# Zehong-Ma/MagCache

Hardware: NVIDIA H100
Metric: denoising_steps_per_sec (higher is better)
Workload: dtype bf16

## Files before the change

### magcache_b200/csrc/gemm_wgmma.cu

```cuda
#include <cstdlib>

#include "common.cuh"
#include "ptx.cuh"
#include "tma_host.cuh"

namespace mc {

TmapCacheEntry* tmap_cache() {
  static TmapCacheEntry table[kTmapCacheSize] = {};
  return table;
}
std::mutex& tmap_cache_mutex() {
  static std::mutex m;
  return m;
}

constexpr int kBM = 128, kBK = 64, kStages = 4;
constexpr int kTileABytes = kBM * kBK * 2;
constexpr int kStagePad = 33;
constexpr int kEpiWarps = 8;
constexpr int kStagingBytes = kEpiWarps * 32 * kStagePad * 4;
constexpr int kGemmThreads = 128 + 32 * kEpiWarps;
constexpr int kProducerRegs = 40, kConsumerRegs = 232;
template <int BN>
struct GemmTile {
  static constexpr int kTileBBytes = BN * kBK * 2;
  static constexpr int kStageBytes = kTileABytes + kTileBBytes;
  static constexpr int kOffStaging = kStages * kStageBytes;
  static constexpr int kOffBars = kOffStaging + kStagingBytes;
  static constexpr int kSmem = kOffBars + 128;
};

struct GemmParams {
  int M, N, K;
  const float* bias;
  void* out;
  int64_t ldo;
  const float* gate;
  int total_tiles;
};

template <int EPI>
__device__ __forceinline__ void epilogue_patch(const GemmParams& p, const float* stage, int row0, int col0, int lane) {
  const int rows = min(32, p.M - row0);
  if (rows <= 0) return;
  const int col = col0 + lane;
  const bool col_ok = col < p.N;

  if (EPI == MC_EPI_BIAS_GATE_RESID) {
    const float b = (p.bias && col_ok) ? p.bias[col] : 0.f;
    const float g = (p.gate && col_ok) ? p.gate[col] : 1.f;
    float* xcol = static_cast<float*>(p.out) + static_cast<int64_t>(row0) * p.ldo + col;
#pragma unroll
    for (int h = 0; h < 32; h += 16) {
      float xv[16];
#pragma unroll
      for (int r = 0; r < 16; ++r) xv[r] = (col_ok && h + r < rows) ? xcol[static_cast<int64_t>(h + r) * p.ldo] : 0.f;
#pragma unroll
      for (int r = 0; r < 16; ++r) {
        const float y = round_bf16(stage[(h + r) * kStagePad + lane] + b);
        xv[r] = __fadd_rn(xv[r], __fmul_rn(y, g));
      }
#pragma unroll
      for (int r = 0; r < 16; ++r)
        if (col_ok && h + r < rows) xcol[static_cast<int64_t>(h + r) * p.ldo] = xv[r];
    }
    return;
  }

  if (EPI == MC_EPI_BIAS_F32) {
    const float b = (p.bias && col_ok) ? p.bias[col] : 0.f;
    float* ocol = static_cast<float*>(p.out) + static_cast<int64_t>(row0) * p.ldo + col;
#pragma unroll
    for (int r = 0; r < 32; ++r)
      if (col_ok && r < rows) ocol[static_cast<int64_t>(r) * p.ldo] = stage[r * kStagePad + lane] + b;
    return;
  }

  const int half = lane >> 4, cp = (lane & 15) * 2;
  const int c0 = col0 + cp;
  float b0 = 0.f, b1 = 0.f;
  if (EPI != MC_EPI_ROWBIAS_BF16 && p.bias) {
    if (c0 < p.N) b0 = p.bias[c0];
    if (c0 + 1 < p.N) b1 = p.bias[c0 + 1];
  }
  float g0 = 1.f, g1 = 1.f;
  if (EPI == MC_EPI_BIAS_GATE_RESID_BF16 && p.gate) {
    if (c0 < p.N) g0 = p.gate[c0];
    if (c0 + 1 < p.N) g1 = p.gate[c0 + 1];
  }
  __nv_bfloat16* obase = static_cast<__nv_bfloat16*>(p.out) + static_cast<int64_t>(row0 + half) * p.ldo + c0;
  const float* sbase = stage + half * kStagePad + cp;
  const float* rbias = (EPI == MC_EPI_ROWBIAS_BF16 && p.bias) ? p.bias + row0 + half : nullptr;

  if (rows == 32 && col0 + 32 <= p.N && (p.ldo & 1) == 0) {
    uint32_t w[16];
#pragma unroll
    for (int i = 0; i < 16; ++i) {
      float v0 = sbase[2 * i * kStagePad], v1 = sbase[2 * i * kStagePad + 1];
      if (EPI == MC_EPI_ROWBIAS_BF16) {
        const float rb = rbias ? rbias[2 * i] : 0.f;
        v0 += rb;
        v1 += rb;
      } else {
        v0 += b0;
        v1 += b1;
      }
      if (EPI == MC_EPI_BIAS_GELU_BF16) {
        v0 = gelu_tanh(round_bf16(v0));
        v1 = gelu_tanh(round_bf16(v1));
      }
      if (EPI == MC_EPI_BIAS_GELU_ERF_BF16) {
        v0 = gelu_erf(round_bf16(v0));
        v1 = gelu_erf(round_bf16(v1));
      }
      if (EPI == MC_EPI_BIAS_SILU_BF16) {
        v0 = silu_f(round_bf16(v0));
        v1 = silu_f(round_bf16(v1));
      }
      if (EPI == MC_EPI_BIAS_GATE_RESID_BF16) {
        const uint32_t old = *reinterpret_cast<const uint32_t*>(obase + static_cast<int64_t>(2 * i) * p.ldo);
        v0 = bf16_lo(old) + round_bf16(g0 * round_bf16(v0));
        v1 = bf16_hi(old) + round_bf16(g1 * round_bf16(v1));
      }
      w[i] = pack_bf16x2(v0, v1);
    }
#pragma unroll
    for (int i = 0; i < 16; ++i) *reinterpret_cast<uint32_t*>(obase + static_cast<int64_t>(2 * i) * p.ldo) = w[i];
    return;
  }

  const bool pair_ok = (c0 + 1 < p.N) && ((p.ldo & 1) == 0);
  for (int i = 0; i < 16; ++i) {
    const int r = 2 * i + half;
    if (r >= rows) continue;
    float v0 = sbase[2 * i * kStagePad], v1 = sbase[2 * i * kStagePad + 1];
    if (EPI == MC_EPI_ROWBIAS_BF16) {
      const float rb = rbias ? rbias[2 * i] : 0.f;
      v0 += rb;
      v1 += rb;
    } else {
      v0 += b0;
      v1 += b1;
    }
    if (EPI == MC_EPI_BIAS_GELU_BF16) {
      v0 = gelu_tanh(round_bf16(v0));
      v1 = gelu_tanh(round_bf16(v1));
    }
    if (EPI == MC_EPI_BIAS_GELU_ERF_BF16) {
      v0 = gelu_erf(round_bf16(v0));
      v1 = gelu_erf(round_bf16(v1));
    }
    if (EPI == MC_EPI_BIAS_SILU_BF16) {
      v0 = silu_f(round_bf16(v0));
      v1 = silu_f(round_bf16(v1));
    }
    __nv_bfloat16* o = obase + static_cast<int64_t>(2 * i) * p.ldo;
    if (EPI == MC_EPI_BIAS_GATE_RESID_BF16) {
      if (c0 < p.N) v0 = __bfloat162float(o[0]) + round_bf16(g0 * round_bf16(v0));
      if (c0 + 1 < p.N) v1 = __bfloat162float(o[1]) + round_bf16(g1 * round_bf16(v1));
    }
    if (pair_ok) {
      *reinterpret_cast<uint32_t*>(o) = pack_bf16x2(v0, v1);
    } else {
      if (c0 < p.N) o[0] = __float2bfloat16_rn(v0);
      if (c0 + 1 < p.N) o[1] = __float2bfloat16_rn(v1);
    }
  }
}

template <int EPI, int kBN>
__global__ void __launch_bounds__(kGemmThreads, 1)
    gemm_bf16_kernel(const __grid_constant__ CUtensorMap tmap_a, const __grid_constant__ CUtensorMap tmap_b, const GemmParams p) {
  using T = GemmTile<kBN>;
  constexpr int kStageBytes = T::kStageBytes, kOffStaging = T::kOffStaging, kOffBars = T::kOffBars;
  extern __shared__ __align__(1024) uint8_t smem[];
  float* staging = reinterpret_cast<float*>(smem + kOffStaging);
  uint64_t* full_bar = reinterpret_cast<uint64_t*>(smem + kOffBars);
  uint64_t* empty_bar = full_bar + kStages;

  const int warp = threadIdx.x >> 5, lane = threadIdx.x & 31;
  const int n_tiles = (p.N + kBN - 1) / kBN;
  const int total_tiles = p.total_tiles;
  const int num_kb = (p.K + kBK - 1) / kBK;

  if (threadIdx.x == 0) {
    if ((ptx::smem_u32(smem) & 1023u) != 0) {
      MC_DIAG("gemm_bf16_kernel: dynamic smem base not 1024-aligned\n");
      __trap();
    }
    ptx::prefetch_tmap(&tmap_a);
    ptx::prefetch_tmap(&tmap_b);
    for (int s = 0; s < kStages; ++s) {
      ptx::mbar_init(&full_bar[s], 1);
      ptx::mbar_init(&empty_bar[s], kEpiWarps);
    }
    ptx::fence_mbar_init();
  }
  __syncthreads();

  if (warp < 4) {
    ptx::setmaxnreg_dec<kProducerRegs>();
    if (warp == 0) {
      uint32_t it = 0;
      for (int tile = blockIdx.x; tile < total_tiles; tile += gridDim.x) {
        const int m0 = (tile / n_tiles) * kBM, n0 = (tile % n_tiles) * kBN;
        for (int kb = 0; kb < num_kb; ++kb, ++it) {
          const int s = it % kStages;
          const uint32_t ph = (it / kStages) & 1;
          ptx::mbar_wait(&empty_bar[s], ph ^ 1);
          if (ptx::elect_one()) {
            uint8_t* sa = smem + s * kStageBytes;
            ptx::mbar_expect_tx(&full_bar[s], kStageBytes);
            ptx::tma_load_2d(sa, &tmap_a, &full_bar[s], kb * kBK, m0);
            ptx::tma_load_2d(sa + kTileABytes, &tmap_b, &full_bar[s], kb * kBK, n0);
          }
          __syncwarp();
        }
      }
    }
  } else {
    ptx::setmaxnreg_inc<kConsumerRegs>();
    const int wg = (warp >> 2) - 1;
    const int wq = warp & 3;
    float acc[kBN / 2];
    uint32_t it = 0;
    for (int tile = blockIdx.x; tile < total_tiles; tile += gridDim.x) {
      const int m0 = (tile / n_tiles) * kBM, n0 = (tile % n_tiles) * kBN;
      int prev_s = -1;
      for (int kb = 0; kb < num_kb; ++kb, ++it) {
        const int s = it % kStages;
        const uint32_t ph = (it / kStages) & 1;
        ptx::mbar_wait(&full_bar[s], ph);
        const uint32_t sa = ptx::smem_u32(smem + s * kStageBytes);
        const uint64_t da = ptx::gmma_desc_sw128_kmajor(sa + wg * (64 * 128));
        const uint64_t db = ptx::gmma_desc_sw128_kmajor(sa + kTileABytes);
        ptx::wgmma_fence();
#pragma unroll
        for (int k = 0; k < kBK / 16; ++k) {
          if constexpr (kBN == 256) {
            ptx::wgmma_m64n256k16_ss(acc, da + 2 * k, db + 2 * k, (kb | k) != 0 ? 1u : 0u);
          } else {
            ptx::wgmma_m64n128k16_ss(acc, da + 2 * k, db + 2 * k, (kb | k) != 0 ? 1u : 0u);
          }
        }
        ptx::wgmma_commit();
        ptx::wgmma_wait<1>();
        ptx::fence_regs(acc);
        if (prev_s >= 0 && lane == 0) ptx::mbar_arrive(&empty_bar[prev_s]);
        prev_s = s;
      }
      ptx::wgmma_wait<0>();
      ptx::fence_regs(acc);
      if (lane == 0) ptx::mbar_arrive(&empty_bar[prev_s]);

      const int pr = wq >> 1;
      const int row0 = m0 + wg * 64 + pr * 32;
      const int r_lo = (wq & 1) * 16 + (lane >> 2);
#pragma unroll
      for (int c = 0; c < kBN / 32; ++c) {
        float* patch = staging + (4 * wg + 2 * pr + (c & 1)) * 32 * kStagePad;
        asm volatile("bar.sync %0, 64;" ::"r"(1 + 2 * wg + pr) : "memory");
#pragma unroll
        for (int q = 0; q < 4; ++q) {
          const int i = 4 * c + q;
          const int col = 8 * q + 2 * (lane & 3);
          patch[r_lo * kStagePad + col] = acc[4 * i + 0];
          patch[r_lo * kStagePad + col + 1] = acc[4 * i + 1];
          patch[(r_lo + 8) * kStagePad + col] = acc[4 * i + 2];
          patch[(r_lo + 8) * kStagePad + col + 1] = acc[4 * i + 3];
        }
        asm volatile("bar.sync %0, 64;" ::"r"(1 + 2 * wg + pr) : "memory");
        if ((wq & 1) == (c & 1)) epilogue_patch<EPI>(p, patch, row0, n0 + c * 32, lane);
      }
    }
  }
}

template <int EPI, int BN>
static int32_t launch_gemm_bn(const CUtensorMap& ta, const CUtensorMap& tb, GemmParams p, cudaStream_t s) {
  static PerDeviceOnce once;
  const int32_t rc = set_max_smem_once(gemm_bf16_kernel<EPI, BN>, GemmTile<BN>::kSmem, once, "cudaFuncSetAttribute(gemm smem)");
  if (rc) return rc;
  const int m_tiles = (p.M + kBM - 1) / kBM, n_tiles = (p.N + BN - 1) / BN;
  const int total = m_tiles * n_tiles;
  p.total_tiles = total;
  const int grid = total < num_sms() ? total : num_sms();
  gemm_bf16_kernel<EPI, BN><<<grid, kGemmThreads, GemmTile<BN>::kSmem, s>>>(ta, tb, p);
  MC_CHECK_LAUNCH("gemm_bf16_kernel launch");
  return MC_OK;
}

static int pick_bn(int M, int N) {
  const char* e = getenv("MC_GEMM_BN");
  if (e && *e) {
    const int v = atoi(e);
    if (v == 128 || v == 256) return v;
  }
  const int64_t sms = num_sms(), m_tiles = (M + kBM - 1) / kBM;
  const int64_t t256 = m_tiles * ((N + 255) / 256), t128 = m_tiles * ((N + 127) / 128);
  const int64_t cost256 = ((t256 + sms - 1) / sms) * 100, cost128 = ((t128 + sms - 1) / sms) * 62;
  return cost128 * 100 <= cost256 * 92 ? 128 : 256;
}

}

extern "C" int32_t mc_gemm_bf16(const void* A, int64_t lda, const void* B, int64_t ldb, int32_t M, int32_t N, int32_t K,
                                const float* bias, int32_t epilogue, void* out, int64_t ldo, const float* gate, void* stream) {
  MC_CHECK_ARG(A && B && out, "mc_gemm_bf16: null pointer");
  MC_CHECK_ARG(M >= 1 && N >= 1 && K >= 8, "mc_gemm_bf16: M=%d N=%d K=%d", M, N, K);
  MC_CHECK_ARG(K % 8 == 0 && lda % 8 == 0 && ldb % 8 == 0 && lda >= K && ldb >= K, "mc_gemm_bf16: K/lda/ldb must be multiples of 8 (16-byte TMA pitch)");
  MC_CHECK_ARG(mc::aligned16(A) && mc::aligned16(B) && mc::aligned16(out), "mc_gemm_bf16: A/B/out must be 16-byte aligned");
  MC_CHECK_ARG(ldo >= N, "mc_gemm_bf16: ldo=%lld < N=%d", static_cast<long long>(ldo), N);
  CUtensorMap ta, tb;
  int32_t rc = mc::make_tmap_bf16_2d(&ta, A, static_cast<uint64_t>(M), static_cast<uint64_t>(K), static_cast<uint64_t>(lda), mc::kBM, mc::kBK);
  if (rc) return rc;
  const int bn = mc::pick_bn(M, N);
  rc = mc::make_tmap_bf16_2d(&tb, B, static_cast<uint64_t>(N), static_cast<uint64_t>(K), static_cast<uint64_t>(ldb), bn, mc::kBK);
  if (rc) return rc;
  mc::GemmParams p{M, N, K, bias, out, ldo, gate, 0};
  cudaStream_t s = static_cast<cudaStream_t>(stream);
#define MC_GEMM_CASE(E) \
  case E: return bn == 128 ? mc::launch_gemm_bn<E, 128>(ta, tb, p, s) : mc::launch_gemm_bn<E, 256>(ta, tb, p, s)
  switch (epilogue) {
    MC_GEMM_CASE(MC_EPI_BIAS_BF16);
    MC_GEMM_CASE(MC_EPI_BIAS_GELU_BF16);
    MC_GEMM_CASE(MC_EPI_BIAS_GATE_RESID);
    MC_GEMM_CASE(MC_EPI_ROWBIAS_BF16);
    MC_GEMM_CASE(MC_EPI_BIAS_F32);
    MC_GEMM_CASE(MC_EPI_BIAS_GELU_ERF_BF16);
    MC_GEMM_CASE(MC_EPI_BIAS_GATE_RESID_BF16);
    MC_GEMM_CASE(MC_EPI_BIAS_SILU_BF16);
#undef MC_GEMM_CASE
    default:
      mc::set_error("mc_gemm_bf16: unknown epilogue %d", epilogue);
      return MC_ERR_INVALID;
  }
}
```

### magcache_b200/csrc/ptx.cuh

```cuda
#pragma once
#include <cstdint>
#include <cuda_runtime.h>

namespace ptx {

__device__ __forceinline__ uint32_t smem_u32(const void* p) {
  return static_cast<uint32_t>(__cvta_generic_to_shared(p));
}

__device__ __forceinline__ void mbar_init(uint64_t* bar, uint32_t count) {
  asm volatile("mbarrier.init.shared::cta.b64 [%0], %1;" ::"r"(smem_u32(bar)), "r"(count) : "memory");
}
__device__ __forceinline__ void fence_mbar_init() {
  asm volatile("fence.mbarrier_init.release.cluster;" ::: "memory");
}
__device__ __forceinline__ void mbar_expect_tx(uint64_t* bar, uint32_t bytes) {
  asm volatile("mbarrier.arrive.expect_tx.shared::cta.b64 _, [%0], %1;" ::"r"(smem_u32(bar)), "r"(bytes) : "memory");
}
__device__ __forceinline__ void mbar_arrive(uint64_t* bar) {
  asm volatile("mbarrier.arrive.shared::cta.b64 _, [%0];" ::"r"(smem_u32(bar)) : "memory");
}
__device__ __forceinline__ bool mbar_try_wait(uint64_t* bar, uint32_t parity) {
  uint32_t ok;
  asm volatile(
      "{\n"
      ".reg .pred p;\n"
      "mbarrier.try_wait.parity.shared::cta.b64 p, [%1], %2;\n"
      "selp.u32 %0, 1, 0, p;\n"
      "}\n"
      : "=r"(ok)
      : "r"(smem_u32(bar)), "r"(parity)
      : "memory");
  return ok != 0;
}
#ifndef MC_DEVICE_DIAG
#define MC_DEVICE_DIAG 0
#endif
#if MC_DEVICE_DIAG
#define MC_DIAG(...) printf(__VA_ARGS__)
#else
#define MC_DIAG(...) ((void)0)
#endif

#ifndef MC_MBAR_TIMEOUT_CYCLES
#define MC_MBAR_TIMEOUT_CYCLES (4000000000ll)
#endif
__device__ __forceinline__ void mbar_wait(uint64_t* bar, uint32_t parity) {
  if (mbar_try_wait(bar, parity)) return;
  const long long t0 = clock64();
  while (!mbar_try_wait(bar, parity)) {
    if (clock64() - t0 > MC_MBAR_TIMEOUT_CYCLES) {
      MC_DIAG("mbar_wait timeout: block (%d,%d,%d) thread %d bar smem+%u parity %u\n", blockIdx.x, blockIdx.y, blockIdx.z,
              threadIdx.x, smem_u32(bar), parity);
      __trap();
    }
  }
}
__device__ __forceinline__ void mbar_wait_or_flag(uint64_t* bar, uint32_t parity, bool& timed_out) {
  if (timed_out || mbar_try_wait(bar, parity)) return;
  const long long t0 = clock64();
  while (!mbar_try_wait(bar, parity)) {
    if (clock64() - t0 > MC_MBAR_TIMEOUT_CYCLES) {
      MC_DIAG("mbar_wait timeout: block (%d,%d,%d) thread %d bar smem+%u parity %u\n", blockIdx.x, blockIdx.y, blockIdx.z,
              threadIdx.x, smem_u32(bar), parity);
      timed_out = true;
      return;
    }
  }
}

__device__ __forceinline__ void named_bar_sync(uint32_t id, uint32_t count) {
  asm volatile("bar.sync %0, %1;" ::"r"(id), "r"(count) : "memory");
}
__device__ __forceinline__ void named_bar_arrive(uint32_t id, uint32_t count) {
  asm volatile("bar.arrive %0, %1;" ::"r"(id), "r"(count) : "memory");
}

__device__ __forceinline__ bool elect_one() {
  uint32_t pred;
  asm volatile(
      "{\n"
      ".reg .pred P;\n"
      "elect.sync _|P, 0xffffffff;\n"
      "selp.u32 %0, 1, 0, P;\n"
      "}\n"
      : "=r"(pred));
  return pred != 0;
}

__device__ __forceinline__ void fence_proxy_async_smem() {
  asm volatile("fence.proxy.async.shared::cta;" ::: "memory");
}

__device__ __forceinline__ void prefetch_tmap(const void* tmap) {
  asm volatile("prefetch.tensormap [%0];" ::"l"(reinterpret_cast<uint64_t>(tmap)) : "memory");
}
__device__ __forceinline__ void tma_load_2d(void* smem_dst, const void* tmap, uint64_t* bar, int32_t c0, int32_t c1) {
  asm volatile(
      "cp.async.bulk.tensor.2d.shared::cluster.global.mbarrier::complete_tx::bytes [%0], [%1, {%3, %4}], [%2];"
      ::"r"(smem_u32(smem_dst)), "l"(reinterpret_cast<uint64_t>(tmap)), "r"(smem_u32(bar)), "r"(c0), "r"(c1)
      : "memory");
}

__device__ __forceinline__ void bulk_load_1d(void* smem_dst, const void* gmem_src, uint32_t bytes, uint64_t* bar) {
  asm volatile("cp.async.bulk.shared::cluster.global.mbarrier::complete_tx::bytes [%0], [%1], %2, [%3];" ::"r"(smem_u32(smem_dst)),
               "l"(reinterpret_cast<uint64_t>(gmem_src)), "r"(bytes), "r"(smem_u32(bar))
               : "memory");
}

__device__ __forceinline__ uint64_t gmma_desc_sw128_kmajor(uint32_t smem_addr) {
  uint64_t d = 0;
  d |= static_cast<uint64_t>((smem_addr & 0x3FFFFu) >> 4);
  d |= static_cast<uint64_t>(1) << 16;
  d |= static_cast<uint64_t>(1024 >> 4) << 32;
  d |= static_cast<uint64_t>(1) << 62;
  return d;
}
__device__ __forceinline__ uint64_t gmma_desc_sw128_mnmajor(uint32_t smem_addr, uint32_t lbo_bytes, uint32_t sbo_bytes = 1024) {
  uint64_t d = 0;
  d |= static_cast<uint64_t>((smem_addr & 0x3FFFFu) >> 4);
  d |= static_cast<uint64_t>((lbo_bytes >> 4) & 0x3FFFu) << 16;
  d |= static_cast<uint64_t>((sbo_bytes >> 4) & 0x3FFFu) << 32;
  d |= static_cast<uint64_t>(1) << 62;
  return d;
}
__device__ __forceinline__ void wgmma_fence() { asm volatile("wgmma.fence.sync.aligned;" ::: "memory"); }
__device__ __forceinline__ void wgmma_commit() { asm volatile("wgmma.commit_group.sync.aligned;" ::: "memory"); }
template <int N>
__device__ __forceinline__ void wgmma_wait() {
  asm volatile("wgmma.wait_group.sync.aligned %0;" ::"n"(N) : "memory");
}
template <int N>
__device__ __forceinline__ void fence_regs(float (&d)[N]) {
#pragma unroll
  for (int i = 0; i < N; ++i) asm volatile("" : "+f"(d[i])::"memory");
}

__device__ __forceinline__ void wgmma_m64n64k16_ss(float (&d)[32], uint64_t adesc, uint64_t bdesc, uint32_t accumulate) {
  asm volatile(
      "{\n"
      ".reg .pred p;\n"
      "setp.ne.b32 p, %34, 0;\n"
      "wgmma.mma_async.sync.aligned.m64n64k16.f32.bf16.bf16 "
      "{%0, %1, %2, %3, %4, %5, %6, %7, %8, %9, %10, %11, %12, %13, %14, %15, %16, %17, %18, %19, %20, %21, %22, %23, %24, %25, %26, %27, %28, %29, %30, %31}, "
      "%32, %33, p, 1, 1, 0, 0;\n"
      "}\n"
      : "+f"(d[0]), "+f"(d[1]), "+f"(d[2]), "+f"(d[3]), "+f"(d[4]), "+f"(d[5]), "+f"(d[6]), "+f"(d[7]), "+f"(d[8]), "+f"(d[9]), "+f"(d[10]), "+f"(d[11]), "+f"(d[12]), "+f"(d[13]), "+f"(d[14]), "+f"(d[15]), "+f"(d[16]), "+f"(d[17]), "+f"(d[18]), "+f"(d[19]), "+f"(d[20]), "+f"(d[21]), "+f"(d[22]), "+f"(d[23]), "+f"(d[24]), "+f"(d[25]), "+f"(d[26]), "+f"(d[27]), "+f"(d[28]), "+f"(d[29]), "+f"(d[30]), "+f"(d[31])
      : "l"(adesc), "l"(bdesc), "r"(accumulate));
}
__device__ __forceinline__ void wgmma_m64n128k16_ss(float (&d)[64], uint64_t adesc, uint64_t bdesc, uint32_t accumulate) {
  asm volatile(
      "{\n"
      ".reg .pred p;\n"
      "setp.ne.b32 p, %66, 0;\n"
      "wgmma.mma_async.sync.aligned.m64n128k16.f32.bf16.bf16 "
      "{%0, %1, %2, %3, %4, %5, %6, %7, %8, %9, %10, %11, %12, %13, %14, %15, %16, %17, %18, %19, %20, %21, %22, %23, %24, %25, %26, %27, %28, %29, %30, %31, %32, %33, %34, %35, %36, %37, %38, %39, %40, %41, %42, %43, %44, %45, %46, %47, %48, %49, %50, %51, %52, %53, %54, %55, %56, %57, %58, %59, %60, %61, %62, %63}, "
      "%64, %65, p, 1, 1, 0, 0;\n"
      "}\n"
      : "+f"(d[0]), "+f"(d[1]), "+f"(d[2]), "+f"(d[3]), "+f"(d[4]), "+f"(d[5]), "+f"(d[6]), "+f"(d[7]), "+f"(d[8]), "+f"(d[9]), "+f"(d[10]), "+f"(d[11]), "+f"(d[12]), "+f"(d[13]), "+f"(d[14]), "+f"(d[15]), "+f"(d[16]), "+f"(d[17]), "+f"(d[18]), "+f"(d[19]), "+f"(d[20]), "+f"(d[21]), "+f"(d[22]), "+f"(d[23]), "+f"(d[24]), "+f"(d[25]), "+f"(d[26]), "+f"(d[27]), "+f"(d[28]), "+f"(d[29]), "+f"(d[30]), "+f"(d[31]), "+f"(d[32]), "+f"(d[33]), "+f"(d[34]), "+f"(d[35]), "+f"(d[36]), "+f"(d[37]), "+f"(d[38]), "+f"(d[39]), "+f"(d[40]), "+f"(d[41]), "+f"(d[42]), "+f"(d[43]), "+f"(d[44]), "+f"(d[45]), "+f"(d[46]), "+f"(d[47]), "+f"(d[48]), "+f"(d[49]), "+f"(d[50]), "+f"(d[51]), "+f"(d[52]), "+f"(d[53]), "+f"(d[54]), "+f"(d[55]), "+f"(d[56]), "+f"(d[57]), "+f"(d[58]), "+f"(d[59]), "+f"(d[60]), "+f"(d[61]), "+f"(d[62]), "+f"(d[63])
      : "l"(adesc), "l"(bdesc), "r"(accumulate));
}
__device__ __forceinline__ void wgmma_m64n256k16_ss(float (&d)[128], uint64_t adesc, uint64_t bdesc, uint32_t accumulate) {
  asm volatile(
      "{\n"
      ".reg .pred p;\n"
      "setp.ne.b32 p, %130, 0;\n"
      "wgmma.mma_async.sync.aligned.m64n256k16.f32.bf16.bf16 "
      "{%0, %1, %2, %3, %4, %5, %6, %7, %8, %9, %10, %11, %12, %13, %14, %15, %16, %17, %18, %19, %20, %21, %22, %23, %24, %25, %26, %27, %28, %29, %30, %31, %32, %33, %34, %35, %36, %37, %38, %39, %40, %41, %42, %43, %44, %45, %46, %47, %48, %49, %50, %51, %52, %53, %54, %55, %56, %57, %58, %59, %60, %61, %62, %63, %64, %65, %66, %67, %68, %69, %70, %71, %72, %73, %74, %75, %76, %77, %78, %79, %80, %81, %82, %83, %84, %85, %86, %87, %88, %89, %90, %91, %92, %93, %94, %95, %96, %97, %98, %99, %100, %101, %102, %103, %104, %105, %106, %107, %108, %109, %110, %111, %112, %113, %114, %115, %116, %117, %118, %119, %120, %121, %122, %123, %124, %125, %126, %127}, "
      "%128, %129, p, 1, 1, 0, 0;\n"
      "}\n"
      : "+f"(d[0]), "+f"(d[1]), "+f"(d[2]), "+f"(d[3]), "+f"(d[4]), "+f"(d[5]), "+f"(d[6]), "+f"(d[7]), "+f"(d[8]), "+f"(d[9]), "+f"(d[10]), "+f"(d[11]), "+f"(d[12]), "+f"(d[13]), "+f"(d[14]), "+f"(d[15]), "+f"(d[16]), "+f"(d[17]), "+f"(d[18]), "+f"(d[19]), "+f"(d[20]), "+f"(d[21]), "+f"(d[22]), "+f"(d[23]), "+f"(d[24]), "+f"(d[25]), "+f"(d[26]), "+f"(d[27]), "+f"(d[28]), "+f"(d[29]), "+f"(d[30]), "+f"(d[31]), "+f"(d[32]), "+f"(d[33]), "+f"(d[34]), "+f"(d[35]), "+f"(d[36]), "+f"(d[37]), "+f"(d[38]), "+f"(d[39]), "+f"(d[40]), "+f"(d[41]), "+f"(d[42]), "+f"(d[43]), "+f"(d[44]), "+f"(d[45]), "+f"(d[46]), "+f"(d[47]), "+f"(d[48]), "+f"(d[49]), "+f"(d[50]), "+f"(d[51]), "+f"(d[52]), "+f"(d[53]), "+f"(d[54]), "+f"(d[55]), "+f"(d[56]), "+f"(d[57]), "+f"(d[58]), "+f"(d[59]), "+f"(d[60]), "+f"(d[61]), "+f"(d[62]), "+f"(d[63]), "+f"(d[64]), "+f"(d[65]), "+f"(d[66]), "+f"(d[67]), "+f"(d[68]), "+f"(d[69]), "+f"(d[70]), "+f"(d[71]), "+f"(d[72]), "+f"(d[73]), "+f"(d[74]), "+f"(d[75]), "+f"(d[76]), "+f"(d[77]), "+f"(d[78]), "+f"(d[79]), "+f"(d[80]), "+f"(d[81]), "+f"(d[82]), "+f"(d[83]), "+f"(d[84]), "+f"(d[85]), "+f"(d[86]), "+f"(d[87]), "+f"(d[88]), "+f"(d[89]), "+f"(d[90]), "+f"(d[91]), "+f"(d[92]), "+f"(d[93]), "+f"(d[94]), "+f"(d[95]), "+f"(d[96]), "+f"(d[97]), "+f"(d[98]), "+f"(d[99]), "+f"(d[100]), "+f"(d[101]), "+f"(d[102]), "+f"(d[103]), "+f"(d[104]), "+f"(d[105]), "+f"(d[106]), "+f"(d[107]), "+f"(d[108]), "+f"(d[109]), "+f"(d[110]), "+f"(d[111]), "+f"(d[112]), "+f"(d[113]), "+f"(d[114]), "+f"(d[115]), "+f"(d[116]), "+f"(d[117]), "+f"(d[118]), "+f"(d[119]), "+f"(d[120]), "+f"(d[121]), "+f"(d[122]), "+f"(d[123]), "+f"(d[124]), "+f"(d[125]), "+f"(d[126]), "+f"(d[127])
      : "l"(adesc), "l"(bdesc), "r"(accumulate));
}
__device__ __forceinline__ void wgmma_m64n128k16_rs_tb(float (&d)[64], const uint32_t (&a)[4], uint64_t bdesc, uint32_t accumulate) {
  asm volatile(
      "{\n"
      ".reg .pred p;\n"
      "setp.ne.b32 p, %69, 0;\n"
      "wgmma.mma_async.sync.aligned.m64n128k16.f32.bf16.bf16 "
      "{%0, %1, %2, %3, %4, %5, %6, %7, %8, %9, %10, %11, %12, %13, %14, %15, %16, %17, %18, %19, %20, %21, %22, %23, %24, %25, %26, %27, %28, %29, %30, %31, %32, %33, %34, %35, %36, %37, %38, %39, %40, %41, %42, %43, %44, %45, %46, %47, %48, %49, %50, %51, %52, %53, %54, %55, %56, %57, %58, %59, %60, %61, %62, %63}, "
      "{%64, %65, %66, %67}, %68, p, 1, 1, 1;\n"
      "}\n"
      : "+f"(d[0]), "+f"(d[1]), "+f"(d[2]), "+f"(d[3]), "+f"(d[4]), "+f"(d[5]), "+f"(d[6]), "+f"(d[7]), "+f"(d[8]), "+f"(d[9]), "+f"(d[10]), "+f"(d[11]), "+f"(d[12]), "+f"(d[13]), "+f"(d[14]), "+f"(d[15]), "+f"(d[16]), "+f"(d[17]), "+f"(d[18]), "+f"(d[19]), "+f"(d[20]), "+f"(d[21]), "+f"(d[22]), "+f"(d[23]), "+f"(d[24]), "+f"(d[25]), "+f"(d[26]), "+f"(d[27]), "+f"(d[28]), "+f"(d[29]), "+f"(d[30]), "+f"(d[31]), "+f"(d[32]), "+f"(d[33]), "+f"(d[34]), "+f"(d[35]), "+f"(d[36]), "+f"(d[37]), "+f"(d[38]), "+f"(d[39]), "+f"(d[40]), "+f"(d[41]), "+f"(d[42]), "+f"(d[43]), "+f"(d[44]), "+f"(d[45]), "+f"(d[46]), "+f"(d[47]), "+f"(d[48]), "+f"(d[49]), "+f"(d[50]), "+f"(d[51]), "+f"(d[52]), "+f"(d[53]), "+f"(d[54]), "+f"(d[55]), "+f"(d[56]), "+f"(d[57]), "+f"(d[58]), "+f"(d[59]), "+f"(d[60]), "+f"(d[61]), "+f"(d[62]), "+f"(d[63])
      : "r"(a[0]), "r"(a[1]), "r"(a[2]), "r"(a[3]), "l"(bdesc), "r"(accumulate));
}


template <int N>
__device__ __forceinline__ void setmaxnreg_inc() {
  asm volatile("setmaxnreg.inc.sync.aligned.u32 %0;" ::"n"(N));
}
template <int N>
__device__ __forceinline__ void setmaxnreg_dec() {
  asm volatile("setmaxnreg.dec.sync.aligned.u32 %0;" ::"n"(N));
}

__device__ __forceinline__ float ex2_approx(float x) {
  float y;
  asm("ex2.approx.ftz.f32 %0, %1;" : "=f"(y) : "f"(x));
  return y;
}
__device__ __forceinline__ float ex2_emul(float x) {
  const float kMagic = 12582912.0f;
  x = fmaxf(x, -126.0f);
  const float t = __fadd_rd(x, kMagic);
  const float f = x - __fadd_rn(t, -kMagic);
  float p = __fmaf_rn(0.077119089663028717041015625f, f, 0.227564394474029541015625f);
  p = __fmaf_rn(p, f, 0.695146143436431884765625f);
  p = __fmaf_rn(p, f, 1.0f);
  return __int_as_float(__float_as_int(p) + (__float_as_int(t) << 23));
}
__device__ __forceinline__ uint4 ld_nc_v4(const void* p) {
  uint4 r;
  asm volatile("ld.global.nc.L1::no_allocate.v4.u32 {%0, %1, %2, %3}, [%4];" : "=r"(r.x), "=r"(r.y), "=r"(r.z), "=r"(r.w) : "l"(p));
  return r;
}
__device__ __forceinline__ void st_na_v4(void* p, const uint4& v) {
  asm volatile("st.global.L1::no_allocate.v4.u32 [%0], {%1, %2, %3, %4};" ::"l"(p), "r"(v.x), "r"(v.y), "r"(v.z), "r"(v.w) : "memory");
}

__device__ __forceinline__ void ld_nc_v8_f32(const float* p, float (&f)[8]) {
  asm volatile("ld.global.nc.L1::no_allocate.v4.f32 {%0, %1, %2, %3}, [%4];" : "=f"(f[0]), "=f"(f[1]), "=f"(f[2]), "=f"(f[3]) : "l"(p));
  asm volatile("ld.global.nc.L1::no_allocate.v4.f32 {%0, %1, %2, %3}, [%4];" : "=f"(f[4]), "=f"(f[5]), "=f"(f[6]), "=f"(f[7]) : "l"(p + 4));
}
__device__ __forceinline__ void ld_v8_f32(const float* p, float (&f)[8]) {
  asm volatile("ld.global.v4.f32 {%0, %1, %2, %3}, [%4];" : "=f"(f[0]), "=f"(f[1]), "=f"(f[2]), "=f"(f[3]) : "l"(p) : "memory");
  asm volatile("ld.global.v4.f32 {%0, %1, %2, %3}, [%4];" : "=f"(f[4]), "=f"(f[5]), "=f"(f[6]), "=f"(f[7]) : "l"(p + 4) : "memory");
}
__device__ __forceinline__ void st_na_v8_f32(float* p, const float (&f)[8]) {
  asm volatile("st.global.L1::no_allocate.v4.f32 [%0], {%1, %2, %3, %4};" ::"l"(p), "f"(f[0]), "f"(f[1]), "f"(f[2]), "f"(f[3]) : "memory");
  asm volatile("st.global.L1::no_allocate.v4.f32 [%0], {%1, %2, %3, %4};" ::"l"(p + 4), "f"(f[4]), "f"(f[5]), "f"(f[6]), "f"(f[7]) : "memory");
}
}
```

Measured before the change: 1.615.

## Use 2-CTA clusters with TMA multicast of B tiles across M-adjacent CTAs

The GEMM kernel now launches in clusters of two CTAs that share an N tile and cover adjacent M tiles. Each CTA loads half of the B tile and multicasts it to both, which halves the L2/global traffic for B. Empty barriers now wait on arrivals from both CTAs' consumer warps, and the grid is sized with cudaOccupancyMaxActiveClusters. The epilogue also moves from named-barrier 32-row patches to per-warp 16-row patches synced with __syncwarp. In exchange, the CTAs are coupled in lockstep, which can cost throughput, and M tile rounding now happens at 256 rows.

```diff
diff --git a/magcache_b200/csrc/gemm_wgmma.cu b/magcache_b200/csrc/gemm_wgmma.cu
--- a/magcache_b200/csrc/gemm_wgmma.cu
+++ b/magcache_b200/csrc/gemm_wgmma.cu
@@ -15,16 +15,20 @@
   return m;
 }
 
+constexpr int kCluster = 2;
 constexpr int kBM = 128, kBK = 64, kStages = 4;
+constexpr int kClusterBM = kCluster * kBM;
 constexpr int kTileABytes = kBM * kBK * 2;
 constexpr int kStagePad = 33;
 constexpr int kEpiWarps = 8;
-constexpr int kStagingBytes = kEpiWarps * 32 * kStagePad * 4;
+constexpr int kPatchRows = 16;
+constexpr int kStagingBytes = kEpiWarps * kPatchRows * kStagePad * 4;
 constexpr int kGemmThreads = 128 + 32 * kEpiWarps;
 constexpr int kProducerRegs = 40, kConsumerRegs = 232;
 template <int BN>
 struct GemmTile {
   static constexpr int kTileBBytes = BN * kBK * 2;
+  static constexpr int kHalfBBytes = kTileBBytes / kCluster;
   static constexpr int kStageBytes = kTileABytes + kTileBBytes;
   static constexpr int kOffStaging = kStages * kStageBytes;
   static constexpr int kOffBars = kOffStaging + kStagingBytes;
@@ -40,9 +44,9 @@
   int total_tiles;
 };
 
-template <int EPI>
+template <int EPI, int ROWS>
 __device__ __forceinline__ void epilogue_patch(const GemmParams& p, const float* stage, int row0, int col0, int lane) {
-  const int rows = min(32, p.M - row0);
+  const int rows = min(ROWS, p.M - row0);
   if (rows <= 0) return;
   const int col = col0 + lane;
   const bool col_ok = col < p.N;
@@ -52,7 +56,7 @@
     const float g = (p.gate && col_ok) ? p.gate[col] : 1.f;
     float* xcol = static_cast<float*>(p.out) + static_cast<int64_t>(row0) * p.ldo + col;
 #pragma unroll
-    for (int h = 0; h < 32; h += 16) {
+    for (int h = 0; h < ROWS; h += 16) {
       float xv[16];
 #pragma unroll
       for (int r = 0; r < 16; ++r) xv[r] = (col_ok && h + r < rows) ? xcol[static_cast<int64_t>(h + r) * p.ldo] : 0.f;
@@ -72,7 +76,7 @@
     const float b = (p.bias && col_ok) ? p.bias[col] : 0.f;
     float* ocol = static_cast<float*>(p.out) + static_cast<int64_t>(row0) * p.ldo + col;
 #pragma unroll
-    for (int r = 0; r < 32; ++r)
+    for (int r = 0; r < ROWS; ++r)
       if (col_ok && r < rows) ocol[static_cast<int64_t>(r) * p.ldo] = stage[r * kStagePad + lane] + b;
     return;
   }
@@ -93,10 +97,10 @@
   const float* sbase = stage + half * kStagePad + cp;
   const float* rbias = (EPI == MC_EPI_ROWBIAS_BF16 && p.bias) ? p.bias + row0 + half : nullptr;
 
-  if (rows == 32 && col0 + 32 <= p.N && (p.ldo & 1) == 0) {
-    uint32_t w[16];
-#pragma unroll
-    for (int i = 0; i < 16; ++i) {
+  if (rows == ROWS && col0 + 32 <= p.N && (p.ldo & 1) == 0) {
+    uint32_t w[ROWS / 2];
+#pragma unroll
+    for (int i = 0; i < ROWS / 2; ++i) {
       float v0 = sbase[2 * i * kStagePad], v1 = sbase[2 * i * kStagePad + 1];
       if (EPI == MC_EPI_ROWBIAS_BF16) {
         const float rb = rbias ? rbias[2 * i] : 0.f;
@@ -126,12 +130,12 @@
       w[i] = pack_bf16x2(v0, v1);
     }
 #pragma unroll
-    for (int i = 0; i < 16; ++i) *reinterpret_cast<uint32_t*>(obase + static_cast<int64_t>(2 * i) * p.ldo) = w[i];
+    for (int i = 0; i < ROWS / 2; ++i) *reinterpret_cast<uint32_t*>(obase + static_cast<int64_t>(2 * i) * p.ldo) = w[i];
     return;
   }
 
   const bool pair_ok = (c0 + 1 < p.N) && ((p.ldo & 1) == 0);
-  for (int i = 0; i < 16; ++i) {
+  for (int i = 0; i < ROWS / 2; ++i) {
     const int r = 2 * i + half;
     if (r >= rows) continue;
     float v0 = sbase[2 * i * kStagePad], v1 = sbase[2 * i * kStagePad + 1];
@@ -170,7 +174,7 @@
 }
 
 template <int EPI, int kBN>
-__global__ void __launch_bounds__(kGemmThreads, 1)
+__global__ void __cluster_dims__(kCluster, 1, 1) __launch_bounds__(kGemmThreads, 1)
     gemm_bf16_kernel(const __grid_constant__ CUtensorMap tmap_a, const __grid_constant__ CUtensorMap tmap_b, const GemmParams p) {
   using T = GemmTile<kBN>;
   constexpr int kStageBytes = T::kStageBytes, kOffStaging = T::kOffStaging, kOffBars = T::kOffBars;
@@ -181,8 +185,10 @@
 
   const int warp = threadIdx.x >> 5, lane = threadIdx.x & 31;
   const int n_tiles = (p.N + kBN - 1) / kBN;
-  const int total_tiles = p.total_tiles;
   const int num_kb = (p.K + kBK - 1) / kBK;
+  const uint32_t rank = ptx::cluster_ctarank();
+  const int cluster = static_cast<int>(ptx::cluster_id_x()), n_clusters = static_cast<int>(ptx::num_clusters_x());
+  const int steps = (p.total_tiles - cluster + n_clusters - 1) / n_clusters;
 
   if (threadIdx.x == 0) {
     if ((ptx::smem_u32(smem) & 1023u) != 0) {
@@ -193,18 +199,21 @@
     ptx::prefetch_tmap(&tmap_b);
     for (int s = 0; s < kStages; ++s) {
       ptx::mbar_init(&full_bar[s], 1);
-      ptx::mbar_init(&empty_bar[s], kEpiWarps);
+      ptx::mbar_init(&empty_bar[s], kCluster * kEpiWarps);
     }
     ptx::fence_mbar_init();
   }
-  __syncthreads();
+  ptx::cluster_arrive();
+  ptx::cluster_wait();
 
   if (warp < 4) {
     ptx::setmaxnreg_dec<kProducerRegs>();
     if (warp == 0) {
       uint32_t it = 0;
-      for (int tile = blockIdx.x; tile < total_tiles; tile += gridDim.x) {
-        const int m0 = (tile / n_tiles) * kBM, n0 = (tile % n_tiles) * kBN;
+      for (int i = 0; i < steps; ++i) {
+        const int tile = cluster + i * n_clusters;
+        const int m0 = (tile / n_tiles) * kClusterBM + static_cast<int>(rank) * kBM, n0 = (tile % n_tiles) * kBN;
+        const int nb = n0 + static_cast<int>(rank) * (kBN / kCluster);
         for (int kb = 0; kb < num_kb; ++kb, ++it) {
           const int s = it % kStages;
           const uint32_t ph = (it / kStages) & 1;
@@ -213,7 +222,8 @@
             uint8_t* sa = smem + s * kStageBytes;
             ptx::mbar_expect_tx(&full_bar[s], kStageBytes);
             ptx::tma_load_2d(sa, &tmap_a, &full_bar[s], kb * kBK, m0);
-            ptx::tma_load_2d(sa + kTileABytes, &tmap_b, &full_bar[s], kb * kBK, n0);
+            ptx::tma_load_2d_multicast(sa + kTileABytes + rank * T::kHalfBBytes, &tmap_b, &full_bar[s], kb * kBK, nb,
+                                       static_cast<uint16_t>((1u << kCluster) - 1));
           }
           __syncwarp();
         }
@@ -224,14 +234,16 @@
     const int wg = (warp >> 2) - 1;
     const int wq = warp & 3;
     float acc[kBN / 2];
-    uint32_t it = 0;
-    for (int tile = blockIdx.x; tile < total_tiles; tile += gridDim.x) {
-      const int m0 = (tile / n_tiles) * kBM, n0 = (tile % n_tiles) * kBN;
+    bool timed_out = false;
+    for (int i = 0; i < steps; ++i) {
+      const int tile = cluster + i * n_clusters;
+      const int m0 = (tile / n_tiles) * kClusterBM + static_cast<int>(rank) * kBM, n0 = (tile % n_tiles) * kBN;
+      uint32_t it = static_cast<uint32_t>(i) * num_kb;
       int prev_s = -1;
       for (int kb = 0; kb < num_kb; ++kb, ++it) {
         const int s = it % kStages;
         const uint32_t ph = (it / kStages) & 1;
-        ptx::mbar_wait(&full_bar[s], ph);
+        ptx::mbar_wait_or_flag(&full_bar[s], ph, timed_out);
         const uint32_t sa = ptx::smem_u32(smem + s * kStageBytes);
         const uint64_t da = ptx::gmma_desc_sw128_kmajor(sa + wg * (64 * 128));
         const uint64_t db = ptx::gmma_desc_sw128_kmajor(sa + kTileABytes);
@@ -247,20 +259,21 @@
         ptx::wgmma_commit();
         ptx::wgmma_wait<1>();
         ptx::fence_regs(acc);
-        if (prev_s >= 0 && lane == 0) ptx::mbar_arrive(&empty_bar[prev_s]);
+        if (prev_s >= 0 && lane == 0)
+          for (uint32_t c = 0; c < kCluster; ++c) ptx::mbar_arrive_cluster(&empty_bar[prev_s], c);
         prev_s = s;
       }
       ptx::wgmma_wait<0>();
       ptx::fence_regs(acc);
-      if (lane == 0) ptx::mbar_arrive(&empty_bar[prev_s]);
-
-      const int pr = wq >> 1;
-      const int row0 = m0 + wg * 64 + pr * 32;
-      const int r_lo = (wq & 1) * 16 + (lane >> 2);
+      if (lane == 0)
+        for (uint32_t c = 0; c < kCluster; ++c) ptx::mbar_arrive_cluster(&empty_bar[prev_s], c);
+
+      float* patch = staging + (4 * wg + wq) * kPatchRows * kStagePad;
+      const int row0 = m0 + wg * 64 + wq * kPatchRows;
+      const int r_lo = lane >> 2;
 #pragma unroll
       for (int c = 0; c < kBN / 32; ++c) {
-        float* patch = staging + (4 * wg + 2 * pr + (c & 1)) * 32 * kStagePad;
-        asm volatile("bar.sync %0, 64;" ::"r"(1 + 2 * wg + pr) : "memory");
+        __syncwarp();
 #pragma unroll
         for (int q = 0; q < 4; ++q) {
           const int i = 4 * c + q;
@@ -270,22 +283,52 @@
           patch[(r_lo + 8) * kStagePad + col] = acc[4 * i + 2];
           patch[(r_lo + 8) * kStagePad + col + 1] = acc[4 * i + 3];
         }
-        asm volatile("bar.sync %0, 64;" ::"r"(1 + 2 * wg + pr) : "memory");
-        if ((wq & 1) == (c & 1)) epilogue_patch<EPI>(p, patch, row0, n0 + c * 32, lane);
-      }
-    }
-  }
+        __syncwarp();
+        epilogue_patch<EPI, kPatchRows>(p, patch, row0, n0 + c * 32, lane);
+      }
+    }
+    if (timed_out) __trap();
+  }
+  ptx::cluster_arrive();
+  ptx::cluster_wait();
+}
+
+template <int EPI, int BN>
+static int32_t max_active_clusters(int* out) {
+  static int cached[kMaxDevices] = {};
+  const int d = current_device();
+  if (cached[d] > 0) {
+    *out = cached[d];
+    return MC_OK;
+  }
+  cudaLaunchConfig_t cfg = {};
+  cfg.gridDim = dim3(kCluster * num_sms(), 1, 1);
+  cfg.blockDim = dim3(kGemmThreads, 1, 1);
+  cfg.dynamicSmemBytes = GemmTile<BN>::kSmem;
+  int n = 0;
+  const cudaError_t e = cudaOccupancyMaxActiveClusters(&n, gemm_bf16_kernel<EPI, BN>, &cfg);
+  if (e != cudaSuccess) return cuda_fail(e, "cudaOccupancyMaxActiveClusters(gemm)");
+  if (n < 1) {
+    set_error("gemm_bf16_kernel: no cluster of %d CTAs with %d B of shared memory fits on this device", kCluster, GemmTile<BN>::kSmem);
+    return MC_ERR_CUDA;
+  }
+  cached[d] = n;
+  *out = n;
+  return MC_OK;
 }
 
 template <int EPI, int BN>
 static int32_t launch_gemm_bn(const CUtensorMap& ta, const CUtensorMap& tb, GemmParams p, cudaStream_t s) {
   static PerDeviceOnce once;
-  const int32_t rc = set_max_smem_once(gemm_bf16_kernel<EPI, BN>, GemmTile<BN>::kSmem, once, "cudaFuncSetAttribute(gemm smem)");
+  int32_t rc = set_max_smem_once(gemm_bf16_kernel<EPI, BN>, GemmTile<BN>::kSmem, once, "cudaFuncSetAttribute(gemm smem)");
   if (rc) return rc;
-  const int m_tiles = (p.M + kBM - 1) / kBM, n_tiles = (p.N + BN - 1) / BN;
+  int clusters = 0;
+  rc = max_active_clusters<EPI, BN>(&clusters);
+  if (rc) return rc;
+  const int m_tiles = (p.M + kClusterBM - 1) / kClusterBM, n_tiles = (p.N + BN - 1) / BN;
   const int total = m_tiles * n_tiles;
   p.total_tiles = total;
-  const int grid = total < num_sms() ? total : num_sms();
+  const int grid = kCluster * (total < clusters ? total : clusters);
   gemm_bf16_kernel<EPI, BN><<<grid, kGemmThreads, GemmTile<BN>::kSmem, s>>>(ta, tb, p);
   MC_CHECK_LAUNCH("gemm_bf16_kernel launch");
   return MC_OK;
@@ -297,7 +340,7 @@
     const int v = atoi(e);
     if (v == 128 || v == 256) return v;
   }
-  const int64_t sms = num_sms(), m_tiles = (M + kBM - 1) / kBM;
+  const int64_t sms = num_sms(), m_tiles = (M + 127) / 128;
   const int64_t t256 = m_tiles * ((N + 255) / 256), t128 = m_tiles * ((N + 127) / 128);
   const int64_t cost256 = ((t256 + sms - 1) / sms) * 100, cost128 = ((t128 + sms - 1) / sms) * 62;
   return cost128 * 100 <= cost256 * 92 ? 128 : 256;
@@ -316,7 +359,8 @@
   int32_t rc = mc::make_tmap_bf16_2d(&ta, A, static_cast<uint64_t>(M), static_cast<uint64_t>(K), static_cast<uint64_t>(lda), mc::kBM, mc::kBK);
   if (rc) return rc;
   const int bn = mc::pick_bn(M, N);
-  rc = mc::make_tmap_bf16_2d(&tb, B, static_cast<uint64_t>(N), static_cast<uint64_t>(K), static_cast<uint64_t>(ldb), bn, mc::kBK);
+  rc = mc::make_tmap_bf16_2d(&tb, B, static_cast<uint64_t>(N), static_cast<uint64_t>(K), static_cast<uint64_t>(ldb), bn / mc::kCluster,
+                             mc::kBK);
   if (rc) return rc;
   mc::GemmParams p{M, N, K, bias, out, ldo, gate, 0};
   cudaStream_t s = static_cast<cudaStream_t>(stream);
diff --git a/magcache_b200/csrc/ptx.cuh b/magcache_b200/csrc/ptx.cuh
--- a/magcache_b200/csrc/ptx.cuh
+++ b/magcache_b200/csrc/ptx.cuh
@@ -76,6 +76,34 @@
   asm volatile("bar.arrive %0, %1;" ::"r"(id), "r"(count) : "memory");
 }
 
+__device__ __forceinline__ uint32_t cluster_ctarank() {
+  uint32_t r;
+  asm volatile("mov.u32 %0, %%cluster_ctarank;" : "=r"(r));
+  return r;
+}
+__device__ __forceinline__ uint32_t cluster_id_x() {
+  uint32_t r;
+  asm volatile("mov.u32 %0, %%clusterid.x;" : "=r"(r));
+  return r;
+}
+__device__ __forceinline__ uint32_t num_clusters_x() {
+  uint32_t r;
+  asm volatile("mov.u32 %0, %%nclusterid.x;" : "=r"(r));
+  return r;
+}
+__device__ __forceinline__ void mbar_arrive_cluster(uint64_t* bar, uint32_t cta) {
+  asm volatile(
+      "{\n"
+      ".reg .b32 ra;\n"
+      "mapa.shared::cluster.u32 ra, %0, %1;\n"
+      "mbarrier.arrive.shared::cluster.b64 _, [ra];\n"
+      "}\n"
+      ::"r"(smem_u32(bar)), "r"(cta)
+      : "memory");
+}
+__device__ __forceinline__ void cluster_arrive() { asm volatile("barrier.cluster.arrive.release.aligned;" ::: "memory"); }
+__device__ __forceinline__ void cluster_wait() { asm volatile("barrier.cluster.wait.acquire.aligned;" ::: "memory"); }
+
 __device__ __forceinline__ bool elect_one() {
   uint32_t pred;
   asm volatile(
@@ -99,6 +127,14 @@
   asm volatile(
       "cp.async.bulk.tensor.2d.shared::cluster.global.mbarrier::complete_tx::bytes [%0], [%1, {%3, %4}], [%2];"
       ::"r"(smem_u32(smem_dst)), "l"(reinterpret_cast<uint64_t>(tmap)), "r"(smem_u32(bar)), "r"(c0), "r"(c1)
+      : "memory");
+}
+
+__device__ __forceinline__ void tma_load_2d_multicast(void* smem_dst, const void* tmap, uint64_t* bar, int32_t c0, int32_t c1,
+                                                      uint16_t cta_mask) {
+  asm volatile(
+      "cp.async.bulk.tensor.2d.shared::cluster.global.mbarrier::complete_tx::bytes.multicast::cluster [%0], [%1, {%3, %4}], [%2], %5;"
+      ::"r"(smem_u32(smem_dst)), "l"(reinterpret_cast<uint64_t>(tmap)), "r"(smem_u32(bar)), "r"(c0), "r"(c1), "h"(cta_mask)
       : "memory");
 }
 
```

New measurement: 1.677 (median of 6 runs). 3.8% higher.
